# NVlabs/GLAMR

Measured on NVIDIA H100. Metric: global_opt_frame_person_iterations_per_sec, higher is better.
Workload: dtype f32

## Files before the change

### glamr_b200/csrc/common.cuh

```cuda
#pragma once
#include <cuda_fp16.h>
#include <cuda_runtime.h>
#include <stdint.h>
#include <stdio.h>
#include <stdlib.h>

#include "../../include/glamr_b200.h"

#define GLAMR_CUDA_TRY(expr)                       \
  do {                                             \
    cudaError_t _e = (expr);                       \
    if (_e != cudaSuccess) return (int)_e;         \
  } while (0)

#define GLAMR_LAUNCH_CHECK()                       \
  do {                                             \
    cudaError_t _e = cudaGetLastError();           \
    if (_e != cudaSuccess) return (int)_e;         \
  } while (0)

#ifdef GLAMR_EXPERIMENT
#define GLAMR_DBG(x) (x)
#else
#define GLAMR_DBG(x) 0
// ... 171 lines not shown
  asm("cvt.rna.tf32.f32 %0, %1;" : "=r"(h) : "f"(x));
  hi = __uint_as_float(h);
  asm("cvt.rna.tf32.f32 %0, %1;" : "=r"(l) : "f"(x - hi));
  lo = __uint_as_float(l);
}
__device__ __forceinline__ void split_f16_scaled(float x, float s, __half& hi, __half& lo) {
  const float xs = x * s;
  hi = __float2half_rn(xs);
  lo = __float2half_rn(xs - __half2float(hi));
}

__device__ __forceinline__ float warp_sum(float v) {
#pragma unroll
  for (int o = 16; o > 0; o >>= 1) v += __shfl_xor_sync(0xffffffffu, v, o);
  return v;
}
__device__ __forceinline__ double warp_sum(double v) {
#pragma unroll
  for (int o = 16; o > 0; o >>= 1) v += __shfl_xor_sync(0xffffffffu, v, o);
  return v;
}

#if defined(__CUDACC__)
constexpr int kPdlDefaultMask = 0;
inline bool pdl_enabled(int bit) {
  static int mask = -1;
  if (mask < 0) {
    const char* e = getenv("GLAMR_PDL");
    mask = e ? atoi(e) : kPdlDefaultMask;
  }
  return (mask & bit) != 0;
}
template <typename... KArgs, typename... Args>
inline cudaError_t launch_pdl(int bit, void (*kernel)(KArgs...), dim3 grid, dim3 block, size_t smem, cudaStream_t s, Args... args) {
  cudaLaunchConfig_t cfg = {};
  cfg.gridDim = grid;
  cfg.blockDim = block;
  cfg.dynamicSmemBytes = smem;
  cfg.stream = s;
  cudaLaunchAttribute attr[1];
  attr[0].id = cudaLaunchAttributeProgrammaticStreamSerialization;
  attr[0].val.programmaticStreamSerializationAllowed = 1;
  cfg.attrs = attr;
  cfg.numAttrs = pdl_enabled(bit) ? 1 : 0;
  return cudaLaunchKernelEx(&cfg, kernel, KArgs(args)...);
}
#endif
// ... 3 lines not shown
```

### glamr_b200/csrc/globalopt_kernels.cu

```cuda
#include <stdlib.h>
#include <algorithm>
#include <string.h>
#include <vector>

#include "globalopt_frames.cuh"
#include "smpl_model.cuh"
#include "block_scan.cuh"

namespace glamr {

constexpr int kFrameThreads = 128;

struct GroupGrid {
  int res0;
  int cam0;
  int cam30;
  int slot0;
};
struct SlotLayout {
  int res;
  int persons;
  int cam;
  int cam3;
  int n_res, n_cam, n_cam3;
// ... 734 lines not shown
  wo.root_raw += (size_t)n_begin * 3;
  const bool tc = lbs_path() >= 1 && st->smpl.tcB != nullptr;
  SmplWorkspace wo_pose = wo;
  if (tc) {
    wo_pose.tcA = nullptr;
    if (!st->aux) {
      GLAMR_CUDA_TRY(cudaStreamCreateWithFlags(&st->aux, cudaStreamNonBlocking));
      GLAMR_CUDA_TRY(cudaEventCreateWithFlags(&st->ev_fork, cudaEventDisableTiming));
      GLAMR_CUDA_TRY(cudaEventCreateWithFlags(&st->ev_join, cudaEventDisableTiming));
      GLAMR_CUDA_TRY(cudaEventCreateWithFlags(&st->ev_sup, cudaEventDisableTiming));
    }
  }
  const bool split = tc && skin_split(st);
  st->n_ev_side = 0;
  bool forked = false;
#ifdef GLAMR_EXPERIMENT
  static const int exp_skip = getenv("GLAMR_EXP_SKIP") ? atoi(getenv("GLAMR_EXP_SKIP")) : 0;
#else
  constexpr int exp_skip = 0;
#endif
  const float* const pose_l = pb.smpl_pose_all + (size_t)n_begin * 69;
  const float* const beta_l = pb.smpl_beta_all + (size_t)n_begin * kNB;
  const bool features_top = st->features_early && !st->timing;
  auto fork_blend = [&](bool features, bool gemm, cudaEvent_t wait_for = nullptr) -> int {
    if (wait_for) {
      GLAMR_CUDA_TRY(cudaStreamWaitEvent(st->aux, wait_for, 0));
    } else {
      GLAMR_CUDA_TRY(cudaEventRecord(st->ev_fork, s));
      GLAMR_CUDA_TRY(cudaStreamWaitEvent(st->aux, st->ev_fork, 0));
    }
    if (st->timing && features && !split) GLAMR_CUDA_TRY(cudaEventRecord(st->ev_blend0, st->aux));
    if (!(exp_skip & 1)) {
      const int rc = launch_blend(st->smpl, n_end - n_begin, pose_l, beta_l, wo, st->aux, features, gemm);
      if (rc) return rc;
    }
    if (gemm) {
      if (st->timing) GLAMR_CUDA_TRY(cudaEventRecord(st->ev_blend1, st->aux));
      if (st->timing == 2 && split) GLAMR_CUDA_TRY(cudaEventRecord(st->ev_side[st->n_ev_side++], st->aux));
      GLAMR_CUDA_TRY(cudaEventRecord(st->ev_join, st->aux));
      forked = true;
    }
    return GLAMR_OK;
  };
  if (tc && n_end > n_begin) {
    if (!st->vpt_ready) {
      const int rc = launch_blend(st->smpl, n_end - n_begin, pose_l, beta_l, wo, s);
      if (rc) return rc;
      st->vpt_ready = 1;
    }
    if (features_top) {
      const int rc = fork_blend(true, false);
      if (rc) return rc;
    }
  }
  const SlotLayout sl = st->sl;
  const int cam_rows_ctas = (sl.cam_rows + kFrameThreads - 1) / kFrameThreads;
// ... 4 lines not shown
  }
  GLAMR_MARK();
  if (n_end > n_begin) {
    const int nn = n_end - n_begin;
    int rc;
    if ((rc = launch_pose_prep(st->smpl, nn, st->sc.orient_world + (size_t)n_begin * 3, pose_l, beta_l, 1, wo_pose, s, true))) return rc;
    GLAMR_MARK();
    if (split) {
      const int sms = smpl_device_sms(), nft = (nn + kSkF - 1) / kSkF;
      const int sup_ctas = std::min(sms, (st->smpl.sk_tiles - kNVTiles) * nft);
      const int mesh_ctas = std::max(sms - sup_ctas, sms / 2);
      GLAMR_CUDA_TRY(cudaEventRecord(st->ev_fork, s));
      if (st->timing) GLAMR_CUDA_TRY(cudaEventRecord(st->ev_lbs0, s));
      if (!(exp_skip & 2))
        if ((rc = launch_skin(st->smpl, nn, wo, nullptr, s, kNVTiles, st->smpl.sk_tiles, sms))) return rc;
      GLAMR_CUDA_TRY(cudaEventRecord(st->ev_sup, s));
      if (st->timing) GLAMR_CUDA_TRY(cudaEventRecord(st->ev_lbs1, s));
      GLAMR_CUDA_TRY(cudaStreamWaitEvent(st->aux, st->ev_fork, 0));
      if (st->timing) GLAMR_CUDA_TRY(cudaEventRecord(st->ev_blend0, st->aux));
      if (st->timing == 2) GLAMR_CUDA_TRY(cudaEventRecord(st->ev_side[st->n_ev_side++], st->aux));
      if (!(exp_skip & 2))
        if ((rc = launch_skin(st->smpl, nn, wo, nullptr, st->aux, 0, kNVTiles, mesh_ctas))) return rc;
      if (st->timing == 2) GLAMR_CUDA_TRY(cudaEventRecord(st->ev_side[st->n_ev_side++], st->aux));
      if ((rc = fork_blend(!features_top, true, st->ev_sup))) return rc;
    } else if (tc) {
      if (st->timing) GLAMR_CUDA_TRY(cudaEventRecord(st->ev_lbs0, s));
      if (!(exp_skip & 2))
        if ((rc = launch_skin(st->smpl, nn, wo, nullptr, s, 0, kNVTiles, smpl_device_sms()))) return rc;
      if (st->timing) GLAMR_CUDA_TRY(cudaEventRecord(st->ev_lbs1, s));
      if ((rc = fork_blend(!features_top, true))) return rc;
    } else {
      if (st->timing) GLAMR_CUDA_TRY(cudaEventRecord(st->ev_lbs0, s));
      if ((rc = launch_lbs(st->smpl, 0, nn, beta_l, wo, nullptr, s, true))) return rc;
      if (st->timing) GLAMR_CUDA_TRY(cudaEventRecord(st->ev_lbs1, s));
    }
    GLAMR_MARK();
  }
  if (!(exp_skip & 4))
    GLAMR_CUDA_TRY(launch_pdl(8, frame_residuals_kernel, dim3(sl.n_res), dim3(kFrameThreads), 0, s, c, st->smpl, wo, n_begin, st->partial, sl));
  GLAMR_MARK();
  if (from_persons) {
    GLAMR_CUDA_TRY(launch_pdl(16, camera_backward_kernel, dim3(sl.n_cam3), dim3(kFrameThreads), 0, s, c, st->partial, sl));
    GLAMR_CUDA_TRY(launch_pdl(16, camera_scatter_kernel, dim3(cam_rows_ctas), dim3(kFrameThreads), 0, s, c, sl.cam_rows));
    GLAMR_MARK();
  }
  if (!(exp_skip & 8))
    GLAMR_CUDA_TRY(launch_pdl(16, traj_cam_backward_kernel, dim3(pb.P + sl.n_cam), dim3(kScanThreads), 0, s, c, from_persons ? 0 : 1, st->partial,
// ... 136 lines not shown
    st->cap_stride = loss_hist_stride;
  }
  for (; done < n_iters; ++done) GLAMR_CUDA_TRY(cudaGraphLaunch(st->iter_exec, s));
  return GLAMR_OK;
}

extern "C" int glamr_opt_read(glamr_opt_t* st, int what, const float** ptr, size_t* count) {
  if (!st || !ptr || !count) return GLAMR_EINVAL;
  const size_t N = st->N, T = (size_t)st->sl.cam_rows, J = st->pb.J;
  switch (what) {
    case GLAMR_R_ORIENT_WORLD: *ptr = st->sc.orient_world; *count = 3 * N; break;
    case GLAMR_R_TRANS_WORLD: *ptr = st->sc.trans_world; *count = 3 * N; break;
    case GLAMR_R_ORIENT_BASE: *ptr = st->sc.orient_base; *count = 3 * N; break;
    case GLAMR_R_TRANS_BASE: *ptr = st->sc.trans_base; *count = 3 * N; break;
    case GLAMR_R_KP_PRED: *ptr = st->sc.kp_pred; *count = N * J * 2; break;
    case GLAMR_R_ORIENT_CAM_IN_WORLD: *ptr = st->sc.orient_ciw; *count = 3 * N; break;
    case GLAMR_R_TRANS_CAM_IN_WORLD: *ptr = st->sc.trans_ciw; *count = 3 * N; break;
    case GLAMR_R_CAM_POSE: *ptr = st->sc.cam; *count = 12 * T; break;
    case GLAMR_R_CAM_POSE_INV: *ptr = st->sc.cam_inv; *count = 12 * T; break;
    case GLAMR_R_JOINTS_WORLD: *ptr = st->sc.joints_world; *count = N * J * 3; break;
    case GLAMR_R_TRAJ_LOCAL: *ptr = st->sc.traj_local; *count = 11 * N; break;
    case GLAMR_R_ADAM_M: *ptr = st->adam.m; *count = st->pb.n_params; break;
    case GLAMR_R_ADAM_V: *ptr = st->adam.v; *count = st->pb.n_params; break;
    default: return GLAMR_EINVAL;
  }
  return GLAMR_OK;
}
```

### glamr_b200/csrc/smpl_kernels.cu

```cuda
#include <math.h>
#include <algorithm>
#include <cmath>
#include <stdlib.h>
#include <string.h>

#include <vector>

#include "glamr_math.cuh"
#include "smpl_model.cuh"

namespace glamr {

__global__ void __launch_bounds__(128) pose_prep_kernel(SmplDev m, int n, const float* __restrict__ orient,
                                                        const float* __restrict__ body_pose,
                                                        const float* __restrict__ betas, int use_betas, SmplWorkspace w) {
  pdl_launch_dependents();
  pdl_wait();
  const int f = (blockIdx.x * blockDim.x + threadIdx.x) >> 5;
  if (f >= n) return;
  pose_prep_frame(m, f, orient ? orient + (size_t)f * 3 : nullptr, body_pose + (size_t)f * 69, use_betas ? betas + (size_t)f * kNB : nullptr, w,
                  threadIdx.x & 31);
}

constexpr int kFramesPerCta = 32;
// ... 237 lines not shown
        }
      }
    }
  }
}


__global__ void __launch_bounds__(128) blend_features_kernel(int n, const float* __restrict__ body_pose, const float* __restrict__ betas, SmplWorkspace w) {
  const int f = (blockIdx.x * blockDim.x + threadIdx.x) >> 5, lane = threadIdx.x & 31;
  if (f >= n) return;
  float R[9];
  if (lane >= 1 && lane < kNJ) {
    const float* bp = body_pose + (size_t)f * 69 + (lane - 1) * 3;
    const float rv[3] = {bp[0], bp[1], bp[2]};
    rodrigues_smplx(rv, R);
  }
  put_blend_features(w, f, lane, R, betas ? betas + (size_t)f * kNB : nullptr);
}

constexpr int kTcStages = 8;
constexpr int kTcThreads = 288;
constexpr uint32_t kTcABytes = kTcAStageHalves * sizeof(__half);
constexpr uint32_t kTcBBytes = kTcBStageHalves * sizeof(__half);
constexpr size_t kTcRingBytes = (size_t)kTcStages * (kTcABytes + kTcBBytes) + 128;
constexpr size_t kTcSmemBytes = kTcRingBytes + 2 * (size_t)kTcOutCols * kTcOutPitch * sizeof(float);

#ifdef GLAMR_EXPERIMENT
constexpr int kBlendPhaseCtas = 1024;
constexpr int kBlendPhases = 5;
__device__ unsigned long long g_blend_phases[kBlendPhaseCtas][2][kBlendPhases];
#define BLEND_CLOCK_INIT() long long bl_ph[kBlendPhases] = {}; long long bl_t = clock64()
#define BLEND_CLOCK(k) do { const long long bl_now = clock64(); bl_ph[k] += bl_now - bl_t; bl_t = bl_now; } while (0)
#define BLEND_CLOCK_TILE() (++bl_ph[kBlendPhases - 1])
#define BLEND_CLOCK_STORE() do { if ((warp & 3) == 0 && lane == 0 && blockIdx.x < kBlendPhaseCtas)                                     \
      for (int k = 0; k < kBlendPhases; ++k) atomicAdd(&g_blend_phases[blockIdx.x][g][k], (unsigned long long)bl_ph[k]); } while (0)
extern "C" int glamr_exp_blend_phases(long long* out) {
  void* p = nullptr;
  GLAMR_CUDA_TRY(cudaDeviceSynchronize());
  GLAMR_CUDA_TRY(cudaMemcpyFromSymbol(out, g_blend_phases, sizeof(g_blend_phases)));
  GLAMR_CUDA_TRY(cudaGetSymbolAddress(&p, g_blend_phases));
  GLAMR_CUDA_TRY(cudaMemset(p, 0, sizeof(g_blend_phases)));
  return GLAMR_OK;
}
#else
#define BLEND_CLOCK_INIT() do { } while (0)
#define BLEND_CLOCK(k) do { } while (0)
#define BLEND_CLOCK_TILE() do { } while (0)
#define BLEND_CLOCK_STORE() do { } while (0)
#endif

__device__ __forceinline__ void warpgroup_sync(int g) {
  if (g == 0) asm volatile("bar.sync 1, 128;" ::: "memory");
  else asm volatile("bar.sync 2, 128;" ::: "memory");
}

__global__ void __launch_bounds__(kTcThreads, 1) lbs_blend_tc_kernel(SmplDev m, SmplWorkspace w, int mtile0, int mtiles, int half_last, int ntn) {
  extern __shared__ __align__(128) unsigned char tc_raw[];
  __half* As = reinterpret_cast<__half*>(tc_raw);
  __half* Bs = As + kTcStages * kTcAStageHalves;
  uint64_t* full = reinterpret_cast<uint64_t*>(Bs + kTcStages * kTcBStageHalves);
  uint64_t* empty = full + kTcStages;
  const int tid = threadIdx.x, warp = tid >> 5, lane = tid & 31;
  const int ntiles = ntn * mtiles;
  pdl_launch_dependents();
  if (tid == 0) {
#pragma unroll
    for (int s = 0; s < kTcStages; ++s) { mbar_init(&full[s], 1); mbar_init(&empty[s], 8); }
    mbar_fence_init();
  }
  __syncthreads();

  if (warp == 8) {
    if (lane == 0) {
      {
        const __half* gB = m.tcB + (size_t)(blockIdx.x / mtiles) * kTcChunks * kTcBStageHalves;
        for (int c = 0; c < kTcStages; ++c) {
          mbar_expect_tx_only(&full[c], kTcBBytes);
          tma_bulk_g2s(Bs + c * kTcBStageHalves, gB + (size_t)c * kTcBStageHalves, kTcBBytes, &full[c]);
        }
      }
      pdl_wait();
      int q = 0;
      for (int t = blockIdx.x; t < ntiles; t += gridDim.x) {
        const __half* gA = w.tcA + (size_t)(mtile0 + t % mtiles) * kTcChunks * kTcAStageHalves;
        const __half* gB = m.tcB + (size_t)(t / mtiles) * kTcChunks * kTcBStageHalves;
        for (int c = 0; c < kTcChunks; ++c, ++q) {
          const int s = q % kTcStages;
          if (q >= kTcStages) {
            mbar_wait(&empty[s], ((q / kTcStages) - 1) & 1);
            mbar_expect_tx(&full[s], kTcABytes + kTcBBytes);
            tma_bulk_g2s(Bs + s * kTcBStageHalves, gB + (size_t)c * kTcBStageHalves, kTcBBytes, &full[s]);
          } else {
            mbar_expect_tx(&full[s], kTcABytes);
          }
          tma_bulk_g2s(As + s * kTcAStageHalves, gA + (size_t)c * kTcAStageHalves, kTcABytes, &full[s]);
        }
      }
    }
    return;
  }
  const int g = warp >> 2;
  float acc[kTcN / 2];
  float (&acc_half)[kTcN / 4] = *reinterpret_cast<float (*)[kTcN / 4]>(acc);
  float* const vpb = vp_buffer(w);
  const size_t cstride = w.vp_tiled ? (size_t)kSkF : (size_t)w.mpad;
  int q = 0;
  BLEND_CLOCK_INIT();
#pragma unroll 1
  for (int t = blockIdx.x; t < ntiles; t += gridDim.x) {
    const int ntile = t / mtiles, mt = t % mtiles, mtile = mtile0 + mt;
    const bool half = half_last && mt == mtiles - 1;
    const int aoff = half ? 0 : g * 64 * 8, boff = half ? g * 128 * 8 : 0;
    auto mainloop = [&](auto& d, auto mma) {
#pragma unroll 1
      for (int c = 0; c < kTcChunks; ++c, ++q) {
        const int s = q % kTcStages;
        BLEND_CLOCK(3);
        mbar_wait(&full[s], (q / kTcStages) & 1);
        BLEND_CLOCK(0);
        const __half* a = As + s * kTcAStageHalves + aoff;
        const __half* b = Bs + s * kTcBStageHalves + boff;
        const uint64_t dah = wgmma_desc_kmajor_noswizzle(a, kTcM), dal = wgmma_desc_kmajor_noswizzle(a + kTcAStageHalves / 2, kTcM);
        const uint64_t dbh = wgmma_desc_kmajor_noswizzle(b, kTcN), dbl = wgmma_desc_kmajor_noswizzle(b + kTcBStageHalves / 2, kTcN);
        wgmma_fence();
        mma(d, dah, dbh, c > 0 ? 1u : 0u);
        mma(d, dal, dbh, 1u);
        mma(d, dah, dbl, 1u);
        wgmma_commit();
        wgmma_wait<1>();
        if (c > 0 && lane == 0) mbar_arrive(&empty[(q - 1) % kTcStages]);
        BLEND_CLOCK(1);
      }
// ... 14 lines not shown
    for (int h = 0; h < 2; ++h) unscale[h] = w.tcUnscale[f0 + rl + 8 * h] * m.tcB_unscale;
    constexpr int kPieces = kTcOutCols * 16 / 128;
    int soff[kPieces];
    size_t goff[kPieces];
#pragma unroll
    for (int j = 0; j < kPieces; ++j) {
      const int p = (tid & 127) + 128 * j;
      int fq, c;
      if (w.vp_tiled) {
        const int q0 = f0 / 4, grp = (q0 + p / kTcOutCols) / 5;
        const int qa = max(5 * grp - q0, 0), qn = min(5 * grp + 5 - q0, 16) - qa;
        const int pg = p - kTcOutCols * qa;
        c = pg / qn;
        fq = qa + pg - c * qn;
      } else {
        fq = p & 15;
        c = p >> 4;
      }
      const int f = f0 + 4 * fq;
      soff[j] = c * kTcOutPitch + 4 * fq;
      goff[j] = w.vp_tiled ? ((size_t)(f / kSkF) * w.vp_cols + (size_t)(col0 + c)) * kSkF + f % kSkF : (size_t)(col0 + c) * w.mpad + f;
    }
    float* const stage = reinterpret_cast<float*>(tc_raw + kTcRingBytes) + g * kTcOutCols * kTcOutPitch;
#pragma unroll
    for (int k = 0; k < kTcN / kTcOutCols; ++k) {
      if (kTcOutCols * k < ncols) {
        warpgroup_sync(g);
#pragma unroll
        for (int i = 0; i < kTcOutCols / 8; ++i)
#pragma unroll
          for (int h = 0; h < 2; ++h)
#pragma unroll
            for (int e = 0; e < 2; ++e)
              stage[(8 * i + 2 * (lane & 3) + e) * kTcOutPitch + rl + 8 * h] = acc[4 * (k * kTcOutCols / 8 + i) + 2 * h + e] * unscale[h];
        warpgroup_sync(g);
        float* const out = vpb + (size_t)(k * kTcOutCols) * cstride;
#pragma unroll
        for (int j = 0; j < kPieces; ++j)
          *reinterpret_cast<float4*>(out + goff[j]) = *reinterpret_cast<const float4*>(stage + soff[j]);
      }
    }
    BLEND_CLOCK(2);
    BLEND_CLOCK_TILE();
  }
  BLEND_CLOCK_STORE();
}
// ... 122 lines not shown
  return GLAMR_OK;
}
#else
#define SKIN_CLOCK_INIT() do { } while (0)
#define SKIN_CLOCK(k) do { } while (0)
#define SKIN_CLOCK_STORE(items) do { } while (0)
#endif

__global__ void __launch_bounds__(kSkinTcThreads, 1) lbs_skin_tc_kernel(SmplDev m, int n, SmplWorkspace w, float* __restrict__ vertices,
                                                                        int vt0, int vt1) {
  extern __shared__ __align__(128) unsigned char sk_raw[];
  float* Ws = reinterpret_cast<float*>(sk_raw);
  float* Bs = Ws + kSkWImageFloats;
  float* Vs = Bs + 2 * kSkBImageFloats;
  uint64_t* full_w = reinterpret_cast<uint64_t*>(Vs + 2 * kSkVpTileFloats);
  uint64_t* full_b = full_w + 1;
  uint64_t* b_empty = full_w + 3;
  uint64_t* full_v = full_w + 5;
  uint64_t* v_empty = full_w + 7;
  const int tid = threadIdx.x, warp = tid >> 5, lane = tid & 31;
  const int nft = (n + kSkF - 1) / kSkF;
  const int items = (vt1 - vt0) * nft;
  const int i0 = (int)((long long)blockIdx.x * items / gridDim.x), i1 = (int)((long long)(blockIdx.x + 1) * items / gridDim.x);
  pdl_launch_dependents();
  if (tid == 0) {
    mbar_init(full_w, 1);
    for (int b = 0; b < 2; ++b) {
      mbar_init(&full_b[b], 1);
      mbar_init(&b_empty[b], 8);
      mbar_init(&full_v[b], 1);
      mbar_init(&v_empty[b], 8);
    }
    mbar_fence_init();
  }
  __syncthreads();

  if (warp == 8) {
    if (lane == 0) {
      mbar_expect_tx(full_w, kSkWBytes);
      tma_bulk_g2s(Ws, m.skW + (size_t)(vt0 + i0 / nft) * kSkWImageFloats, kSkWBytes, full_w);
      pdl_wait();
      const float* const vpb = vp_buffer(w);
      for (int i = i0, it = 0; i < i1; ++i, ++it) {
        const int vtile = vt0 + i / nft, ftile = i - (vtile - vt0) * nft, vb = it & 1;
        const bool new_w = it > 0 && ftile == 0;
        if (it >= 2) mbar_wait(&b_empty[vb], ((it - 2) >> 1) & 1);
        if (new_w) mbar_wait(&b_empty[vb ^ 1], ((it - 1) >> 1) & 1);
        mbar_expect_tx(&full_b[vb], kSkBBytes + (new_w ? kSkWBytes : 0u));
        tma_bulk_g2s(Bs + vb * kSkBImageFloats, w.skB + (size_t)ftile * kSkBImageFloats, kSkBBytes, &full_b[vb]);
        if (new_w) tma_bulk_g2s(Ws, m.skW + (size_t)vtile * kSkWImageFloats, kSkWBytes, &full_b[vb]);
        if (it >= 2) mbar_wait(&v_empty[vb], ((it - 2) >> 1) & 1);
        mbar_expect_tx(&full_v[vb], kSkVBytes);
        tma_bulk_g2s(Vs + vb * kSkVpTileFloats, vpb + ((size_t)ftile * w.vp_cols + (size_t)vtile * kTileCols) * kSkF, kSkVBytes, &full_v[vb]);
      }
    }
    return;
  }
  const int g = warp >> 2, q = lane & 3;
  int jf[3], jrow[3];
  bool jxy[3];
#pragma unroll
  for (int j = 0; j < 3; ++j) {
    const int c0 = 8 * j + 2 * q;
    jf[j] = c0 >= 12 ? 1 : 0;
    jrow[j] = (c0 - 12 * jf[j]) >> 2;
    jxy[j] = (c0 & 3) == 0;
  }
  const bool odd = (q & 1) == 1;
  const int sf[2] = {odd ? jf[2] : jf[0], jf[1]}, srow[2] = {odd ? jrow[2] : jrow[0], jrow[1]};
  SKIN_CLOCK_INIT();
  mbar_wait(full_w, 0);
  for (int i = i0, it = 0; i < i1; ++i, ++it) {
    const int vtile = vt0 + i / nft, ftile = i - (vtile - vt0) * nft, vb = it & 1;
    const bool sup = vtile >= kNVTiles;
    float* const out = sup ? w.vcompact : vertices;
    const int fstride = sup ? m.S * 3 : kV * 3;
    int orow[2];
    const float* vrow[2];
#pragma unroll
    for (int h = 0; h < 2; ++h) {
      const int vl = g * 64 + (warp & 3) * 16 + (lane >> 2) + 8 * h;
      const int v = (vtile - (sup ? kNVTiles : 0)) * kVTile + vl;
      orow[h] = out && v < (sup ? m.S : kV) ? v * 3 : -1;
      vrow[h] = Vs + vb * kSkVpTileFloats + (size_t)vl * 3 * kSkF;
    }
    SKIN_CLOCK(4);
    mbar_wait(&full_b[vb], (it >> 1) & 1);
    SKIN_CLOCK(0);
    float acc[kSkN / 2];
#pragma unroll
    for (int k = 0; k < kSkN / 2; ++k) acc[k] = 0.0f;
    wgmma_fence();
#pragma unroll
    for (int c = 0; c < kNJ / 8; ++c) {
      const float* a = Ws + c * 2 * kVTile * 4 + g * 64 * 4;
// ... 117 lines not shown
static int lbs_set_attrs() {
  static bool attrs = false;
  if (!attrs) {
    attrs = true;
    GLAMR_CUDA_TRY(cudaFuncSetAttribute(lbs_blend_tc_kernel, cudaFuncAttributePreferredSharedMemoryCarveout, cudaSharedmemCarveoutMaxShared));
    GLAMR_CUDA_TRY(cudaFuncSetAttribute(lbs_skin_tc_kernel, cudaFuncAttributePreferredSharedMemoryCarveout, cudaSharedmemCarveoutMaxShared));
    GLAMR_CUDA_TRY(cudaFuncSetAttribute(blend_features_kernel, cudaFuncAttributePreferredSharedMemoryCarveout, cudaSharedmemCarveoutMaxShared));
    GLAMR_CUDA_TRY(cudaFuncSetAttribute(pose_prep_kernel, cudaFuncAttributePreferredSharedMemoryCarveout, cudaSharedmemCarveoutMaxShared));
    GLAMR_CUDA_TRY(cudaFuncSetAttribute(lbs_blend_tc_kernel, cudaFuncAttributeMaxDynamicSharedMemorySize, (int)kTcSmemBytes));
    GLAMR_CUDA_TRY(cudaFuncSetAttribute(lbs_skin_kernel<4>, cudaFuncAttributeMaxDynamicSharedMemorySize, (int)kSkinSmemBytes));
    GLAMR_CUDA_TRY(cudaFuncSetAttribute(lbs_skin_kernel<0>, cudaFuncAttributeMaxDynamicSharedMemorySize, (int)kSkinSmemBytes));
    GLAMR_CUDA_TRY(cudaFuncSetAttribute(lbs_skin_tc_kernel, cudaFuncAttributeMaxDynamicSharedMemorySize, (int)kSkinTcSmemBytes));
  }
  return GLAMR_OK;
}
int smpl_device_sms() {
  static int sms = 0;
  if (sms <= 0) {
    int dev = 0;
    if (cudaGetDevice(&dev) != cudaSuccess || cudaDeviceGetAttribute(&sms, cudaDevAttrMultiProcessorCount, dev) != cudaSuccess || sms <= 0) sms = 132;
  }
  return sms;
}
static int launch_blend_gemm(const SmplDev& m, int n, const SmplWorkspace& w, cudaStream_t s, bool pdl) {
  const int mtiles = (n + kTcM - 1) / kTcM;
  const int half_last = (n - (mtiles - 1) * kTcM <= kTcM / 2) ? 1 : 0;
  const int ntn = w.vp_tiled ? m.tc_ntiles : kTcNTiles;
  const dim3 grid(min(smpl_device_sms(), ntn * mtiles));
  if (pdl) {
    GLAMR_CUDA_TRY(launch_pdl(4, lbs_blend_tc_kernel, grid, dim3(kTcThreads), kTcSmemBytes, s, m, w, 0, mtiles, half_last, ntn));
    return GLAMR_OK;
  }
  lbs_blend_tc_kernel<<<grid, kTcThreads, kTcSmemBytes, s>>>(m, w, 0, mtiles, half_last, ntn);
  GLAMR_LAUNCH_CHECK();
  return GLAMR_OK;
}
static int launch_skin_tc(const SmplDev& m, int n, const SmplWorkspace& w, float* vertices, cudaStream_t s, bool pdl, int vt0, int vt1,
                          int max_ctas) {
  if (vt1 <= vt0) return GLAMR_OK;
  const dim3 grid(max(1, min(max_ctas, (vt1 - vt0) * ((n + kSkF - 1) / kSkF))));
  if (pdl) {
    GLAMR_CUDA_TRY(launch_pdl(4, lbs_skin_tc_kernel, grid, dim3(kSkinTcThreads), kSkinTcSmemBytes, s, m, n, w, vertices, vt0, vt1));
    return GLAMR_OK;
  }
  lbs_skin_tc_kernel<<<grid, kSkinTcThreads, kSkinTcSmemBytes, s>>>(m, n, w, vertices, vt0, vt1);
  GLAMR_LAUNCH_CHECK();
  return GLAMR_OK;
}
int launch_blend(const SmplDev& m, int n, const float* body_pose, const float* betas, const SmplWorkspace& w, cudaStream_t s, bool features,
                 bool gemm) {
  if (n <= 0) return GLAMR_OK;
  int rc;
  if ((rc = lbs_set_attrs())) return rc;
  if (features) {
    blend_features_kernel<<<(n + 3) / 4, 128, 0, s>>>(n, body_pose, betas, w);
    GLAMR_LAUNCH_CHECK();
  }
  if (gemm) return launch_blend_gemm(m, n, w, s, false);
  return GLAMR_OK;
}
int launch_skin(const SmplDev& m, int n, const SmplWorkspace& w, float* vertices, cudaStream_t s, int vt0, int vt1, int max_ctas) {
  if (n <= 0) return GLAMR_OK;
  int rc;
  if ((rc = lbs_set_attrs())) return rc;
  if (w.vp_tiled) return launch_skin_tc(m, n, w, vertices, s, false, vt0, vt1, max_ctas);
  dim3 grid(kNVTiles, (n + kFramesPerCta - 1) / kFramesPerCta);
  if (m.K == 4) lbs_skin_kernel<4><<<grid, kLbsThreads, kSkinSmemBytes, s>>>(m, 0, n, w, vertices);
  else lbs_skin_kernel<0><<<grid, kLbsThreads, kSkinSmemBytes, s>>>(m, 0, n, w, vertices);
  GLAMR_LAUNCH_CHECK();
  return GLAMR_OK;
}

static int g_lbs_path = -1;
int lbs_path() {
  if (g_lbs_path < 0) {
    const char* e = getenv("GLAMR_LBS_PATH");
    g_lbs_path = e ? (strcmp(e, "tc") == 0 ? 2 : strcmp(e, "tcblend") == 0 ? 1 : 0) : GLAMR_DEFAULT_LBS_TC;
  }
  return g_lbs_path;
}
int lbs_kernel_count(const SmplDev& m) { return (lbs_path() >= 1 && m.tcB) ? 2 : 1; }

int launch_lbs(const SmplDev& m, int n_begin, int n_end, const float* betas, const SmplWorkspace& w, float* vertices, cudaStream_t s,
               bool pdl) {
  if (n_end <= n_begin) return GLAMR_OK;
  if (n_begin % kFramesPerCta != 0) return GLAMR_EINVAL;
  dim3 grid(kNVTiles, (n_end - n_begin + kFramesPerCta - 1) / kFramesPerCta);
  const int path = lbs_path();
  {
    const int rc = lbs_set_attrs();
    if (rc) return rc;
  }
  if (path >= 1 && m.tcB && w.tcA && n_begin == 0) {
    int rc;
    if ((rc = launch_blend_gemm(m, n_end, w, s, pdl))) return rc;
    if (w.vp_tiled) return launch_skin_tc(m, n_end, w, vertices, s, pdl, 0, m.sk_tiles, smpl_device_sms());
    if (pdl) {
      if (m.K == 4) GLAMR_CUDA_TRY(launch_pdl(4, lbs_skin_kernel<4>, grid, dim3(kLbsThreads), kSkinSmemBytes, s, m, n_begin, n_end, w, vertices));
      else GLAMR_CUDA_TRY(launch_pdl(4, lbs_skin_kernel<0>, grid, dim3(kLbsThreads), kSkinSmemBytes, s, m, n_begin, n_end, w, vertices));
    } else {
      if (m.K == 4) lbs_skin_kernel<4><<<grid, kLbsThreads, kSkinSmemBytes, s>>>(m, n_begin, n_end, w, vertices);
      else lbs_skin_kernel<0><<<grid, kLbsThreads, kSkinSmemBytes, s>>>(m, n_begin, n_end, w, vertices);
      GLAMR_LAUNCH_CHECK();
    }
    return GLAMR_OK;
  }
  static int stages = 0, dbg = 0;
  if (!stages) {
    const char* e = getenv("GLAMR_LBS_STAGES");
    stages = (e && atoi(e) == 4) ? 4 : 3;
#ifdef GLAMR_EXPERIMENT
    const char* d = getenv("GLAMR_LBS_DEBUG");
    dbg = d ? atoi(d) : 0;
#endif
    GLAMR_CUDA_TRY(cudaFuncSetAttribute(lbs_kernel<4, 3>, cudaFuncAttributeMaxDynamicSharedMemorySize, (int)lbs_smem_bytes(3)));
    GLAMR_CUDA_TRY(cudaFuncSetAttribute(lbs_kernel<0, 3>, cudaFuncAttributeMaxDynamicSharedMemorySize, (int)lbs_smem_bytes(3)));
    GLAMR_CUDA_TRY(cudaFuncSetAttribute(lbs_kernel<4, 4>, cudaFuncAttributeMaxDynamicSharedMemorySize, (int)lbs_smem_bytes(4)));
  }
// ... 236 lines not shown
    case 2: return m->dev.n_map;
    default: return GLAMR_EINVAL;
  }
}

extern "C" size_t glamr_smpl_workspace_bytes(const glamr_smpl_t* m, int n) {
  if (!m || n < 0) return 0;
  return smpl_workspace_floats(n, m->dev.S) * sizeof(float);
}

extern "C" size_t glamr_smpl_fk_workspace_bytes(const glamr_smpl_t* m, int n) {
  if (!m || n < 0) return 0;
  return smpl_workspace_floats_fk(n, m->dev.S) * sizeof(float);
}

extern "C" int glamr_smpl_forward(const glamr_smpl_t* m, int n, const float* global_orient, const float* body_pose,
                                  const float* betas, const float* root_trans, const float* root_scale, int orig_joints,
                                  float* joints, float* vertices, void* workspace, size_t workspace_bytes, void* stream) {
  if (!m || n < 0 || !body_pose || !betas || !joints || !workspace) return GLAMR_EINVAL;
  if (workspace_bytes < glamr_smpl_workspace_bytes(m, n)) return GLAMR_ENOSPACE;
  if (n == 0) return GLAMR_OK;
  cudaStream_t s = (cudaStream_t)stream;
  const SmplWorkspace w = smpl_carve_workspace(workspace, n, m->dev.S);
  int rc;
  if ((rc = launch_pose_prep(m->dev, n, global_orient, body_pose, betas, 1, w, s))) return rc;
  if ((rc = launch_lbs(m->dev, 0, n, betas, w, vertices, s))) return rc;
  if ((rc = launch_joints_finalize(m->dev, n, orig_joints, root_trans, root_scale, w, joints, s))) return rc;
  if (vertices && root_trans)
    if ((rc = launch_reroot_vertices(n, w.root_raw, root_trans, root_scale, vertices, s))) return rc;
  return GLAMR_OK;
}

extern "C" int glamr_smpl_fk24(const glamr_smpl_t* m, int n, const float* global_orient, const float* body_pose,
                               const float* root_trans, const float* root_scale, float* joints, void* workspace,
                               size_t workspace_bytes, void* stream) {
  if (!m || n < 0 || !body_pose || !joints || !workspace) return GLAMR_EINVAL;
  if (workspace_bytes < glamr_smpl_fk_workspace_bytes(m, n)) return GLAMR_ENOSPACE;
  if (n == 0) return GLAMR_OK;
  cudaStream_t s = (cudaStream_t)stream;
  SmplWorkspace w = smpl_carve_workspace(workspace, n, m->dev.S);
  w.tcA = nullptr;
  w.skB = nullptr;
  w.vp_tiled = 0;
  int rc = launch_pose_prep(m->dev, n, global_orient, body_pose, nullptr, 0, w, s);
  if (rc) return rc;
  fk24_finalize_kernel<<<(n * kNJ * 3 + 255) / 256, 256, 0, s>>>(n, w.jposed, root_trans, root_scale, joints);
  GLAMR_LAUNCH_CHECK();
  return GLAMR_OK;
}
```

### glamr_b200/csrc/smpl_model.cuh

```cuda
#pragma once
#include "common.cuh"
#include "glamr_math.cuh"

namespace glamr {

struct SmplDev {
  const float* pd_tiles;
  const __half* tcB;
  float tcB_unscale;
  int tc_ntiles;
  const float* skW;
  int sk_tiles;
  const float* v_template;
  const float* shapedirs;
  const float* j_template;
  const float* j_shapedirs;
  const float* skin_w;
  const uint8_t* skin_j;
  int K;
  const int32_t* compact_of_vertex;
  int S;
  const int32_t* reg_ptr;
  const int32_t* reg_ci;
  const float* reg_w;
// ... 1 lines not shown
  const int32_t* joint_map;
  int n_extra, n_picks, n_map;
  int parents[kNJ];
  int level[kNJ];
  int n_levels;
};

struct SmplWorkspace {
  float* A;
  float* pf;
  float* jposed;
  float* vcompact;
  float* root_raw;
  __half* tcA;
  float* tcUnscale;
  float* vpT;
  int mpad;
  float* skB;
  float* vpT2;
  const double* flip_src;
  int flip_add;
  int vp_tiled;
  int vp_cols;
};

inline int smpl_sup_tiles(int S) { return (S + kVTile - 1) / kVTile; }
inline int smpl_vp_cols(int S) { return (kTcCols + smpl_sup_tiles(S) * kTileCols + kTcN - 1) / kTcN * kTcN; }

inline size_t smpl_workspace_floats_fk(int n, int S) {
  const size_t n32 = ((size_t)n + 31) / 32 * 32;
  return (size_t)n * (kNJ * 3 + (size_t)S * 3 + 3) + n32 * (kPFPad + kNJ * 12) + 64 + 64;
}
inline size_t smpl_workspace_floats(int n, int S) {
  const size_t n32 = ((size_t)n + 31) / 32 * 32;
  const size_t n128 = ((size_t)n + kTcM - 1) / kTcM * kTcM;
  return (size_t)n * (kNJ * 3 + (size_t)S * 3 + 3) + n32 * (kPFPad + kNJ * 12) + 64 + 64 +
         (n128 / kTcM) * kTcChunks * kTcAStageHalves / 2 + n128 + (size_t)smpl_vp_cols(S) * ((n128 + kSkF - 1) / kSkF * kSkF) +
         ((n128 + kSkF - 1) / kSkF) * kSkBImageFloats + 64;
}
int lbs_path();
inline SmplWorkspace smpl_carve_workspace(void* base, int n, int S) {
  SmplWorkspace w;
  float* p = (float*)base;
  w.A = p; p += ((size_t)n + 31) / 32 * 32 * kNJ * 12;
  w.pf = p; p += ((size_t)n + 31) / 32 * 32 * kPFPad;
  w.jposed = p; p += (size_t)n * kNJ * 3;
  w.vcompact = p; p += (size_t)n * S * 3;
  w.root_raw = p; p += (size_t)n * 3;
  p = (float*)(((uintptr_t)p + 255) & ~(uintptr_t)255);
  w.mpad = (int)(((size_t)n + kTcM - 1) / kTcM * kTcM);
  w.tcA = reinterpret_cast<__half*>(p); p += (size_t)(w.mpad / kTcM) * kTcChunks * kTcAStageHalves / 2;
  w.tcUnscale = p; p += w.mpad;
  w.skB = p; p += (size_t)((w.mpad + kSkF - 1) / kSkF) * kSkBImageFloats;
  w.vpT = p;
  w.vp_tiled = lbs_path() == 2 ? 1 : 0;
  w.vp_cols = smpl_vp_cols(S);
  w.vpT2 = nullptr; w.flip_src = nullptr; w.flip_add = 0;
  return w;
}

#if defined(__CUDACC__)
__device__ __forceinline__ float* vp_buffer(const SmplWorkspace& w) {
  if (!w.vpT2) return w.vpT;
  return ((((int)*w.flip_src) + w.flip_add) & 1) ? w.vpT2 : w.vpT;
}
__device__ __forceinline__ void put_blend_features(const SmplWorkspace& w, int f, int lane, const float* R, const float* __restrict__ beta) {
  float m = 2.0f;
  if (beta) {
#pragma unroll
    for (int l = 0; l < kNB; ++l) m = fmaxf(m, fabsf(beta[l]));
  }
  const int e = 14 - ((int)((__float_as_uint(m) >> 23) & 0xFF) - 127);
  const float scale = ldexpf(1.0f, e);
  __half* tile = w.tcA + (size_t)(f >> 7) * kTcChunks * kTcAStageHalves;
  const int r = f & 127;
  auto put = [&](int k, float v) {
    __half hi, lo;
    split_f16_scaled(v, scale, hi, lo);
    __half* q = tile + (size_t)(k >> 4) * kTcAStageHalves + (((k >> 3) & 1) * kTcM + r) * 8 + (k & 7);
    q[0] = hi;
// ... 97 lines not shown
    float4* A = reinterpret_cast<float4*>(w.A + (((size_t)(f >> 5) * kNJ + j) * 32 + (f & 31)) * 12);
#pragma unroll
    for (int i = 0; i < 3; ++i) A[i] = make_float4(GR[i * 3 + 0], GR[i * 3 + 1], GR[i * 3 + 2], Gt[i] - GJ[i]);
    if (w.vp_tiled) {
      float* img = w.skB + (size_t)(f / kSkF) * kSkBImageFloats + ((size_t)(j >> 2) * kSkN + (f % kSkF) * 12) * 4 + (j & 3);
#pragma unroll
      for (int i = 0; i < 12; ++i) {
        const float v = (i & 3) < 3 ? GR[(i >> 2) * 3 + (i & 3)] : Gt[i >> 2] - GJ[i >> 2];
        float hi, lo;
        split_tf32(v, hi, lo);
        img[i * 4] = hi;
        img[kSkBHalf + i * 4] = lo;
      }
    }
  }
}
#endif

int launch_pose_prep(const SmplDev& m, int n, const float* orient, const float* body_pose, const float* betas,
                     int use_betas, const SmplWorkspace& w, cudaStream_t s, bool pdl = false);
int launch_lbs(const SmplDev& m, int n_begin, int n_end, const float* betas, const SmplWorkspace& w, float* vertices,
               cudaStream_t s, bool pdl = false);
int launch_blend(const SmplDev& m, int n, const float* body_pose, const float* betas, const SmplWorkspace& w, cudaStream_t s,
                 bool features = true, bool gemm = true);
int launch_skin(const SmplDev& m, int n, const SmplWorkspace& w, float* vertices, cudaStream_t s, int vt0, int vt1, int max_ctas);
int smpl_device_sms();
int lbs_kernel_count(const SmplDev& m);
int launch_joints_finalize(const SmplDev& m, int n, int orig_joints, const float* root_trans, const float* root_scale,
                           const SmplWorkspace& w, float* joints, cudaStream_t s);
int launch_reroot_vertices(int n, const float* root_raw, const float* root_trans, const float* root_scale,
                           float* vertices, cudaStream_t s);

}

struct glamr_smpl {
  glamr::SmplDev dev;
  void* allocs[16];
  int n_allocs;
};
```

### glamr_b200/lib.py

```python
import ctypes
import os
import subprocess

import torch

HERE = os.path.dirname(os.path.abspath(__file__))
REL_SO_PATH = os.path.join(HERE, 'libglamr_b200.so')
SO_PATH = os.environ.get('GLAMR_B200_SO') or REL_SO_PATH
EXP_SO_PATH = os.path.join(HERE, 'libglamr_b200_exp.so')
CSRC = os.path.join(HERE, 'csrc')
SOURCES = ['smpl_kernels.cu', 'globalopt_kernels.cu', 'c_api.cu', 'nets_kernels.cu', 'eval_kernels.cu', 'init_kernels.cu']
NUM_TERMS = 21

TERM_INDEX = {
    'kp_2d': 0, 'kp_2d_dist': 1, 'cam_traj_rot': 2, 'cam_traj_trans': 3, 'traj_rot_smoothness': 4,
    'traj_trans_smoothness': 5, 'rel_transform': 6, 'local_traj_dxy_reg': 7, 'local_traj_dheading_reg': 8,
    'local_traj_dheading_reg_new': 9, 'local_traj_rot_reg': 10, 'local_traj_z_reg': 11, 'traj_rot_res': 12,
    'traj_trans_res': 13, 'cam_inv_trans_residual_reg': 14, 'cam_inv_rot_smoothness': 15, 'cam_origin_smoothness': 16,
    'cam_up_reg': 17, 'cam_rot_smoothness': 18, 'cam_trans_smoothness': 19, 'cam_depth_smoothness': 20,
}
CAM_CONST, CAM_PER_FRAME, CAM_FIXED, CAM_FROM_PERSONS = 0, 1, 2, 3
TRAJ_PREDICTED, TRAJ_BASE = 0, 1
(R_ORIENT_WORLD, R_TRANS_WORLD, R_ORIENT_BASE, R_TRANS_BASE, R_KP_PRED, R_ORIENT_CIW, R_TRANS_CIW, R_CAM_POSE,
 R_CAM_POSE_INV, R_JOINTS_WORLD, R_TRAJ_LOCAL, R_ADAM_M, R_ADAM_V) = range(13)

(ROP_AA_TO_ROTMAT, ROP_RODRIGUES_SMPLX, ROP_ROT6D_TO_ROTMAT, ROP_ROTMAT_TO_QUAT, ROP_QUAT_TO_AA, ROP_AA_TO_QUAT,
 ROP_QUAT_MUL, ROP_ROTMAT_TO_AA, ROP_QUAT_TO_ROTMAT, ROP_SAFE_ATAN2, ROP_PROJECT, ROP_MAT3_MUL) = range(12)
ROP_DIMS = {0: (3, 0, 9), 1: (3, 0, 9), 2: (6, 0, 9), 3: (9, 0, 4), 4: (4, 0, 3), 5: (3, 0, 4), 6: (4, 4, 4), 7: (9, 0, 3),
            8: (4, 0, 9), 9: (2, 0, 1), 10: (3, 9, 2), 11: (9, 9, 9)}

FILL_F32, FILL_F64, FILL_F32_W64 = 0, 1, 2

_fp = ctypes.POINTER(ctypes.c_float)
_vp = ctypes.c_void_p


class Person(ctypes.Structure):
    _fields_ = [(n, ctypes.c_int32) for n in
                ['start', 'len', 'group', 'off_xy', 'off_heading', 'off_dxy', 'off_dheading', 'off_z', 'off_rot',
                 'off_world_dheading', 'off_orient_res', 'off_trans_res', 'off_world_dxy', 'off_p2c_rot', 'off_p2c_trans']] + \
               [(n, _vp) for n in
                ['traj_local_pred', 'orient_base_init', 'trans_base_init', 'cam_K', 'kp_target', 'orient_cam_6d',
                 'orient_cam_q', 'trans_cam', 'person2cam', 'dheading_mask', 'rot_mask', 'vis', 'kp_w', 'kp_dist_mask', 'ctr_w', 'ctt_w',
                 'world_dxy_base']]


class Group(ctypes.Structure):
# ... 144 lines not shown
```

### include/glamr_b200.h

```cpp
#ifndef GLAMR_B200_H
#define GLAMR_B200_H

#include <stddef.h>
#include <stdint.h>

#ifdef __cplusplus
extern "C" {
#endif

#define GLAMR_OK 0
#define GLAMR_EINVAL (-1)
#define GLAMR_ENOSPACE (-2)
#define GLAMR_EUNSUPPORTED (-3)

#define GLAMR_NUM_VERTS 6890
#define GLAMR_NUM_JOINTS 24
#define GLAMR_NUM_BETAS 10
#define GLAMR_NUM_POSE_FEAT 207

int glamr_version(void);
int glamr_device_sm_count(void);
int glamr_fp32_probe(int iters, float* scratch, size_t scratch_floats, double* flops, void* stream);

typedef struct glamr_smpl glamr_smpl_t;
// ... 193 lines not shown
                      int n_iters, int use_graph, void* stream);
int glamr_opt_losses(glamr_opt_t* st, const float* reduce_buf, float* loss_terms, void* stream);

int glamr_opt_backward_for_apply(glamr_opt_t* st, const float* theta, float* reduce_buf, void* stream);
int glamr_opt_kernel_timing(glamr_opt_t* st, int enable);
int glamr_opt_last_lbs_parts_ms(glamr_opt_t* st, float* critical_ms, float* blend_ms);
int glamr_opt_time_blend(glamr_opt_t* st, int reps, float* ms);
int glamr_opt_last_lbs_ms(glamr_opt_t* st, float* ms);
int glamr_opt_kernel_times(glamr_opt_t* st, float* ms, int* n);

enum glamr_read {
  GLAMR_R_ORIENT_WORLD = 0,
  GLAMR_R_TRANS_WORLD = 1,
  GLAMR_R_ORIENT_BASE = 2,
  GLAMR_R_TRANS_BASE = 3,
  GLAMR_R_KP_PRED = 4,
  GLAMR_R_ORIENT_CAM_IN_WORLD = 5,
  GLAMR_R_TRANS_CAM_IN_WORLD = 6,
  GLAMR_R_CAM_POSE = 7,
  GLAMR_R_CAM_POSE_INV = 8,
  GLAMR_R_JOINTS_WORLD = 9,
  GLAMR_R_TRAJ_LOCAL = 10,
  GLAMR_R_ADAM_M = 11,
  GLAMR_R_ADAM_V = 12
};
#define GLAMR_MAX_PEERS 8
int glamr_peer_alloc(size_t bytes, void** dev_ptr, unsigned char* ipc_handle_64_bytes);
int glamr_peer_open(const unsigned char* ipc_handle_64_bytes, void** dev_ptr);
int glamr_peer_close(void* dev_ptr);
int glamr_peer_free(void* dev_ptr);
size_t glamr_opt_peer_bytes(const glamr_opt_t* st);
int glamr_opt_set_peers(glamr_opt_t* st, int rank, int world, void* const* bufs );
int glamr_allreduce_inplace(glamr_opt_t* st, float* buf, size_t count, void* stream);

int glamr_sparse_regress(int n, int V, int rows, const int32_t* row_ptr, const int32_t* col_idx, const float* weights,
                         const float* vertices, float* out, void* stream);
int glamr_procrustes_align(int n, int J, const float* S1, const float* S2, float* out, void* stream);

int glamr_opt_read(glamr_opt_t* st, int what, const float** ptr, size_t* count);

#ifdef __cplusplus
}
#endif
#endif
```

Measured before the change: 2.914 million.

## Overlap blend GEMM behind skin via PDL and dynamic tile tickets

The blend tensor-core GEMM launched behind the split skin kernel now uses programmatic dependent launch with bit 64 enabled by default, and defers its grid-dependency wait until the first output store. Its producer warp also switches from static strided tile assignment to an atomic ticket counter, with tile ids passed through shared memory to the consumer warps. The skin kernel triggers dependents only near its last work item. The aim is to hide launch latency and let the GEMM's loads run ahead of the skin kernel finishing, at the cost of added atomics, self-resetting counters that must stay consistent across launches, and a new workspace slot plus a debug read enum.

```diff
diff --git a/glamr_b200/csrc/common.cuh b/glamr_b200/csrc/common.cuh
--- a/glamr_b200/csrc/common.cuh
+++ b/glamr_b200/csrc/common.cuh
@@ -217,7 +217,7 @@
 }
 
 #if defined(__CUDACC__)
-constexpr int kPdlDefaultMask = 0;
+constexpr int kPdlDefaultMask = 64;
 inline bool pdl_enabled(int bit) {
   static int mask = -1;
   if (mask < 0) {
diff --git a/glamr_b200/csrc/globalopt_kernels.cu b/glamr_b200/csrc/globalopt_kernels.cu
--- a/glamr_b200/csrc/globalopt_kernels.cu
+++ b/glamr_b200/csrc/globalopt_kernels.cu
@@ -780,7 +780,7 @@
   const float* const pose_l = pb.smpl_pose_all + (size_t)n_begin * 69;
   const float* const beta_l = pb.smpl_beta_all + (size_t)n_begin * kNB;
   const bool features_top = st->features_early && !st->timing;
-  auto fork_blend = [&](bool features, bool gemm, cudaEvent_t wait_for = nullptr) -> int {
+  auto fork_blend = [&](bool features, bool gemm, cudaEvent_t wait_for = nullptr, bool behind_skin = false) -> int {
     if (wait_for) {
       GLAMR_CUDA_TRY(cudaStreamWaitEvent(st->aux, wait_for, 0));
     } else {
@@ -789,7 +789,7 @@
     }
     if (st->timing && features && !split) GLAMR_CUDA_TRY(cudaEventRecord(st->ev_blend0, st->aux));
     if (!(exp_skip & 1)) {
-      const int rc = launch_blend(st->smpl, n_end - n_begin, pose_l, beta_l, wo, st->aux, features, gemm);
+      const int rc = launch_blend(st->smpl, n_end - n_begin, pose_l, beta_l, wo, st->aux, features, gemm, behind_skin);
       if (rc) return rc;
     }
     if (gemm) {
@@ -840,7 +840,7 @@
       if (!(exp_skip & 2))
         if ((rc = launch_skin(st->smpl, nn, wo, nullptr, st->aux, 0, kNVTiles, mesh_ctas))) return rc;
       if (st->timing == 2) GLAMR_CUDA_TRY(cudaEventRecord(st->ev_side[st->n_ev_side++], st->aux));
-      if ((rc = fork_blend(!features_top, true, st->ev_sup))) return rc;
+      if ((rc = fork_blend(!features_top, true, st->ev_sup, true))) return rc;
     } else if (tc) {
       if (st->timing) GLAMR_CUDA_TRY(cudaEventRecord(st->ev_lbs0, s));
       if (!(exp_skip & 2))
@@ -1023,6 +1023,7 @@
     case GLAMR_R_TRAJ_LOCAL: *ptr = st->sc.traj_local; *count = 11 * N; break;
     case GLAMR_R_ADAM_M: *ptr = st->adam.m; *count = st->pb.n_params; break;
     case GLAMR_R_ADAM_V: *ptr = st->adam.v; *count = st->pb.n_params; break;
+    case GLAMR_R_SMPL_WORKSPACE: *ptr = st->ws.A; *count = smpl_workspace_floats((int)N, st->smpl.S); break;
     default: return GLAMR_EINVAL;
   }
   return GLAMR_OK;
diff --git a/glamr_b200/csrc/smpl_kernels.cu b/glamr_b200/csrc/smpl_kernels.cu
--- a/glamr_b200/csrc/smpl_kernels.cu
+++ b/glamr_b200/csrc/smpl_kernels.cu
@@ -283,7 +283,7 @@
 constexpr int kTcThreads = 288;
 constexpr uint32_t kTcABytes = kTcAStageHalves * sizeof(__half);
 constexpr uint32_t kTcBBytes = kTcBStageHalves * sizeof(__half);
-constexpr size_t kTcRingBytes = (size_t)kTcStages * (kTcABytes + kTcBBytes) + 128;
+constexpr size_t kTcRingBytes = (size_t)kTcStages * (kTcABytes + kTcBBytes) + 128 + 64;
 constexpr size_t kTcSmemBytes = kTcRingBytes + 2 * (size_t)kTcOutCols * kTcOutPitch * sizeof(float);
 
 #ifdef GLAMR_EXPERIMENT
@@ -315,12 +315,14 @@
   else asm volatile("bar.sync 2, 128;" ::: "memory");
 }
 
-__global__ void __launch_bounds__(kTcThreads, 1) lbs_blend_tc_kernel(SmplDev m, SmplWorkspace w, int mtile0, int mtiles, int half_last, int ntn) {
+__global__ void __launch_bounds__(kTcThreads, 1) lbs_blend_tc_kernel(SmplDev m, SmplWorkspace w, int mtile0, int mtiles, int half_last, int ntn,
+                                                                     int wait_at_store) {
   extern __shared__ __align__(128) unsigned char tc_raw[];
   __half* As = reinterpret_cast<__half*>(tc_raw);
   __half* Bs = As + kTcStages * kTcAStageHalves;
   uint64_t* full = reinterpret_cast<uint64_t*>(Bs + kTcStages * kTcBStageHalves);
   uint64_t* empty = full + kTcStages;
+  int* tile_slot = reinterpret_cast<int*>(empty + kTcStages);
   const int tid = threadIdx.x, warp = tid >> 5, lane = tid & 31;
   const int ntiles = ntn * mtiles;
   pdl_launch_dependents();
@@ -333,22 +335,28 @@
 
   if (warp == 8) {
     if (lane == 0) {
-      {
-        const __half* gB = m.tcB + (size_t)(blockIdx.x / mtiles) * kTcChunks * kTcBStageHalves;
+      int t = (int)atomicAdd(&w.tickets[0], 1u);
+      if (t < ntiles) {
+        const __half* gB = m.tcB + (size_t)(t / mtiles) * kTcChunks * kTcBStageHalves;
         for (int c = 0; c < kTcStages; ++c) {
           mbar_expect_tx_only(&full[c], kTcBBytes);
           tma_bulk_g2s(Bs + c * kTcBStageHalves, gB + (size_t)c * kTcBStageHalves, kTcBBytes, &full[c]);
         }
       }
-      pdl_wait();
+      if (!wait_at_store) pdl_wait();
       int q = 0;
-      for (int t = blockIdx.x; t < ntiles; t += gridDim.x) {
+      for (;; t = (int)atomicAdd(&w.tickets[0], 1u)) {
         const __half* gA = w.tcA + (size_t)(mtile0 + t % mtiles) * kTcChunks * kTcAStageHalves;
         const __half* gB = m.tcB + (size_t)(t / mtiles) * kTcChunks * kTcBStageHalves;
         for (int c = 0; c < kTcChunks; ++c, ++q) {
           const int s = q % kTcStages;
+          if (q >= kTcStages) mbar_wait(&empty[s], ((q / kTcStages) - 1) & 1);
+          if (c == 0) tile_slot[s] = t < ntiles ? t : -1;
+          if (t >= ntiles) {
+            mbar_arrive(&full[s]);
+            break;
+          }
           if (q >= kTcStages) {
-            mbar_wait(&empty[s], ((q / kTcStages) - 1) & 1);
             mbar_expect_tx(&full[s], kTcABytes + kTcBBytes);
             tma_bulk_g2s(Bs + s * kTcBStageHalves, gB + (size_t)c * kTcBStageHalves, kTcBBytes, &full[s]);
           } else {
@@ -356,6 +364,12 @@
           }
           tma_bulk_g2s(As + s * kTcAStageHalves, gA + (size_t)c * kTcAStageHalves, kTcABytes, &full[s]);
         }
+        if (t >= ntiles) break;
+      }
+      __threadfence();
+      if (atomicAdd(&w.tickets[1], 1u) == gridDim.x - 1) {
+        atomicExch(&w.tickets[0], 0u);
+        atomicExch(&w.tickets[1], 0u);
       }
     }
     return;
@@ -366,9 +380,13 @@
   float* const vpb = vp_buffer(w);
   const size_t cstride = w.vp_tiled ? (size_t)kSkF : (size_t)w.mpad;
   int q = 0;
+  bool store_wait = wait_at_store != 0;
   BLEND_CLOCK_INIT();
 #pragma unroll 1
-  for (int t = blockIdx.x; t < ntiles; t += gridDim.x) {
+  for (;;) {
+    mbar_wait(&full[q % kTcStages], (q / kTcStages) & 1);
+    const int t = tile_slot[q % kTcStages];
+    if (t < 0) break;
     const int ntile = t / mtiles, mt = t % mtiles, mtile = mtile0 + mt;
     const bool half = half_last && mt == mtiles - 1;
     const int aoff = half ? 0 : g * 64 * 8, boff = half ? g * 128 * 8 : 0;
@@ -429,6 +447,10 @@
       goff[j] = w.vp_tiled ? ((size_t)(f / kSkF) * w.vp_cols + (size_t)(col0 + c)) * kSkF + f % kSkF : (size_t)(col0 + c) * w.mpad + f;
     }
     float* const stage = reinterpret_cast<float*>(tc_raw + kTcRingBytes) + g * kTcOutCols * kTcOutPitch;
+    if (store_wait) {
+      pdl_wait();
+      store_wait = false;
+    }
 #pragma unroll
     for (int k = 0; k < kTcN / kTcOutCols; ++k) {
       if (kTcOutCols * k < ncols) {
@@ -597,7 +619,7 @@
   const int nft = (n + kSkF - 1) / kSkF;
   const int items = (vt1 - vt0) * nft;
   const int i0 = (int)((long long)blockIdx.x * items / gridDim.x), i1 = (int)((long long)(blockIdx.x + 1) * items / gridDim.x);
-  pdl_launch_dependents();
+  if (i1 - i0 <= 1) pdl_launch_dependents();
   if (tid == 0) {
     mbar_init(full_w, 1);
     for (int b = 0; b < 2; ++b) {
@@ -617,6 +639,7 @@
       pdl_wait();
       const float* const vpb = vp_buffer(w);
       for (int i = i0, it = 0; i < i1; ++i, ++it) {
+        if (i == i1 - 1 && it > 0) pdl_launch_dependents();
         const int vtile = vt0 + i / nft, ftile = i - (vtile - vt0) * nft, vb = it & 1;
         const bool new_w = it > 0 && ftile == 0;
         if (it >= 2) mbar_wait(&b_empty[vb], ((it - 2) >> 1) & 1);
@@ -646,6 +669,7 @@
   SKIN_CLOCK_INIT();
   mbar_wait(full_w, 0);
   for (int i = i0, it = 0; i < i1; ++i, ++it) {
+    if (i == i1 - 1 && it > 0) pdl_launch_dependents();
     const int vtile = vt0 + i / nft, ftile = i - (vtile - vt0) * nft, vb = it & 1;
     const bool sup = vtile >= kNVTiles;
     float* const out = sup ? w.vcompact : vertices;
@@ -809,16 +833,17 @@
   }
   return sms;
 }
-static int launch_blend_gemm(const SmplDev& m, int n, const SmplWorkspace& w, cudaStream_t s, bool pdl) {
+static int launch_blend_gemm(const SmplDev& m, int n, const SmplWorkspace& w, cudaStream_t s, int pdl_bit, bool wait_at_store = false) {
   const int mtiles = (n + kTcM - 1) / kTcM;
   const int half_last = (n - (mtiles - 1) * kTcM <= kTcM / 2) ? 1 : 0;
   const int ntn = w.vp_tiled ? m.tc_ntiles : kTcNTiles;
   const dim3 grid(min(smpl_device_sms(), ntn * mtiles));
-  if (pdl) {
-    GLAMR_CUDA_TRY(launch_pdl(4, lbs_blend_tc_kernel, grid, dim3(kTcThreads), kTcSmemBytes, s, m, w, 0, mtiles, half_last, ntn));
+  if (pdl_bit) {
+    GLAMR_CUDA_TRY(launch_pdl(pdl_bit, lbs_blend_tc_kernel, grid, dim3(kTcThreads), kTcSmemBytes, s, m, w, 0, mtiles, half_last, ntn,
+                              wait_at_store ? 1 : 0));
     return GLAMR_OK;
   }
-  lbs_blend_tc_kernel<<<grid, kTcThreads, kTcSmemBytes, s>>>(m, w, 0, mtiles, half_last, ntn);
+  lbs_blend_tc_kernel<<<grid, kTcThreads, kTcSmemBytes, s>>>(m, w, 0, mtiles, half_last, ntn, 0);
   GLAMR_LAUNCH_CHECK();
   return GLAMR_OK;
 }
@@ -835,7 +860,7 @@
   return GLAMR_OK;
 }
 int launch_blend(const SmplDev& m, int n, const float* body_pose, const float* betas, const SmplWorkspace& w, cudaStream_t s, bool features,
-                 bool gemm) {
+                 bool gemm, bool behind_skin) {
   if (n <= 0) return GLAMR_OK;
   int rc;
   if ((rc = lbs_set_attrs())) return rc;
@@ -843,7 +868,7 @@
     blend_features_kernel<<<(n + 3) / 4, 128, 0, s>>>(n, body_pose, betas, w);
     GLAMR_LAUNCH_CHECK();
   }
-  if (gemm) return launch_blend_gemm(m, n, w, s, false);
+  if (gemm) return launch_blend_gemm(m, n, w, s, behind_skin ? 64 : 0, behind_skin && !features);
   return GLAMR_OK;
 }
 int launch_skin(const SmplDev& m, int n, const SmplWorkspace& w, float* vertices, cudaStream_t s, int vt0, int vt1, int max_ctas) {
@@ -880,7 +905,7 @@
   }
   if (path >= 1 && m.tcB && w.tcA && n_begin == 0) {
     int rc;
-    if ((rc = launch_blend_gemm(m, n_end, w, s, pdl))) return rc;
+    if ((rc = launch_blend_gemm(m, n_end, w, s, pdl ? 4 : 0))) return rc;
     if (w.vp_tiled) return launch_skin_tc(m, n_end, w, vertices, s, pdl, 0, m.sk_tiles, smpl_device_sms());
     if (pdl) {
       if (m.K == 4) GLAMR_CUDA_TRY(launch_pdl(4, lbs_skin_kernel<4>, grid, dim3(kLbsThreads), kSkinSmemBytes, s, m, n_begin, n_end, w, vertices));
@@ -1163,6 +1188,7 @@
   if (n == 0) return GLAMR_OK;
   cudaStream_t s = (cudaStream_t)stream;
   const SmplWorkspace w = smpl_carve_workspace(workspace, n, m->dev.S);
+  GLAMR_CUDA_TRY(cudaMemsetAsync(w.tickets, 0, kLbsTickets * sizeof(unsigned int), s));
   int rc;
   if ((rc = launch_pose_prep(m->dev, n, global_orient, body_pose, betas, 1, w, s))) return rc;
   if ((rc = launch_lbs(m->dev, 0, n, betas, w, vertices, s))) return rc;
@@ -1183,6 +1209,7 @@
   w.tcA = nullptr;
   w.skB = nullptr;
   w.vp_tiled = 0;
+  w.tickets = nullptr;
   int rc = launch_pose_prep(m->dev, n, global_orient, body_pose, nullptr, 0, w, s);
   if (rc) return rc;
   fk24_finalize_kernel<<<(n * kNJ * 3 + 255) / 256, 256, 0, s>>>(n, w.jposed, root_trans, root_scale, joints);
diff --git a/glamr_b200/csrc/smpl_model.cuh b/glamr_b200/csrc/smpl_model.cuh
--- a/glamr_b200/csrc/smpl_model.cuh
+++ b/glamr_b200/csrc/smpl_model.cuh
@@ -47,7 +47,9 @@
   int flip_add;
   int vp_tiled;
   int vp_cols;
+  unsigned int* tickets;
 };
+constexpr int kLbsTickets = 2;
 
 inline int smpl_sup_tiles(int S) { return (S + kVTile - 1) / kVTile; }
 inline int smpl_vp_cols(int S) { return (kTcCols + smpl_sup_tiles(S) * kTileCols + kTcN - 1) / kTcN * kTcN; }
@@ -61,7 +63,7 @@
   const size_t n128 = ((size_t)n + kTcM - 1) / kTcM * kTcM;
   return (size_t)n * (kNJ * 3 + (size_t)S * 3 + 3) + n32 * (kPFPad + kNJ * 12) + 64 + 64 +
          (n128 / kTcM) * kTcChunks * kTcAStageHalves / 2 + n128 + (size_t)smpl_vp_cols(S) * ((n128 + kSkF - 1) / kSkF * kSkF) +
-         ((n128 + kSkF - 1) / kSkF) * kSkBImageFloats + 64;
+         ((n128 + kSkF - 1) / kSkF) * kSkBImageFloats + 64 + 64;
 }
 int lbs_path();
 inline SmplWorkspace smpl_carve_workspace(void* base, int n, int S) {
@@ -81,6 +83,7 @@
   w.vp_tiled = lbs_path() == 2 ? 1 : 0;
   w.vp_cols = smpl_vp_cols(S);
   w.vpT2 = nullptr; w.flip_src = nullptr; w.flip_add = 0;
+  w.tickets = reinterpret_cast<unsigned int*>((float*)base + smpl_workspace_floats(n, S) - 64);
   return w;
 }
 
@@ -224,7 +227,7 @@
 int launch_lbs(const SmplDev& m, int n_begin, int n_end, const float* betas, const SmplWorkspace& w, float* vertices,
                cudaStream_t s, bool pdl = false);
 int launch_blend(const SmplDev& m, int n, const float* body_pose, const float* betas, const SmplWorkspace& w, cudaStream_t s,
-                 bool features = true, bool gemm = true);
+                 bool features = true, bool gemm = true, bool behind_skin = false);
 int launch_skin(const SmplDev& m, int n, const SmplWorkspace& w, float* vertices, cudaStream_t s, int vt0, int vt1, int max_ctas);
 int smpl_device_sms();
 int lbs_kernel_count(const SmplDev& m);
diff --git a/glamr_b200/lib.py b/glamr_b200/lib.py
--- a/glamr_b200/lib.py
+++ b/glamr_b200/lib.py
@@ -22,7 +22,7 @@
 CAM_CONST, CAM_PER_FRAME, CAM_FIXED, CAM_FROM_PERSONS = 0, 1, 2, 3
 TRAJ_PREDICTED, TRAJ_BASE = 0, 1
 (R_ORIENT_WORLD, R_TRANS_WORLD, R_ORIENT_BASE, R_TRANS_BASE, R_KP_PRED, R_ORIENT_CIW, R_TRANS_CIW, R_CAM_POSE,
- R_CAM_POSE_INV, R_JOINTS_WORLD, R_TRAJ_LOCAL, R_ADAM_M, R_ADAM_V) = range(13)
+ R_CAM_POSE_INV, R_JOINTS_WORLD, R_TRAJ_LOCAL, R_ADAM_M, R_ADAM_V, R_SMPL_WORKSPACE) = range(14)
 
 (ROP_AA_TO_ROTMAT, ROP_RODRIGUES_SMPLX, ROP_ROT6D_TO_ROTMAT, ROP_ROTMAT_TO_QUAT, ROP_QUAT_TO_AA, ROP_AA_TO_QUAT,
  ROP_QUAT_MUL, ROP_ROTMAT_TO_AA, ROP_QUAT_TO_ROTMAT, ROP_SAFE_ATAN2, ROP_PROJECT, ROP_MAT3_MUL) = range(12)
diff --git a/include/glamr_b200.h b/include/glamr_b200.h
--- a/include/glamr_b200.h
+++ b/include/glamr_b200.h
@@ -239,7 +239,8 @@
   GLAMR_R_JOINTS_WORLD = 9,
   GLAMR_R_TRAJ_LOCAL = 10,
   GLAMR_R_ADAM_M = 11,
-  GLAMR_R_ADAM_V = 12
+  GLAMR_R_ADAM_V = 12,
+  GLAMR_R_SMPL_WORKSPACE = 13
 };
 #define GLAMR_MAX_PEERS 8
 int glamr_peer_alloc(size_t bytes, void** dev_ptr, unsigned char* ipc_handle_64_bytes);
```

New measurement: 2.975 million (median of 6 runs). +2.1%, better.
